# dominikbuenger/torch_nfft

Measured on AMD Instinct MI355X. Metric: Mpoints/s (adjoint+forward, 3-D N=256 m=4), higher is better.
Workload: dtype f32

## Files before the change

### torch_nfft_amd/csrc/colfft.hip

```cpp
#include <type_traits>

#include "common.h"
#include "kernels.h"

namespace nfft {

namespace {

constexpr int kFftThreads = 256;

struct ColGeom {
    int M, logM, N, H;
    int Mh;
    int SR;
    int KC;
    int KS;
    int NB;
    int NBm;
    int two_d;
    int NC, logNC;
    int TG;
    float param;
};

// ... 72 lines not shown
    static std::atomic<const float2 *> cache[kMaxDevices][7];
    const int dev = current_device();
    int slot = 0;
    while ((16 << slot) < M) ++slot;
    if (slot > 6 || (16 << slot) != M) return nullptr;
    if (dev < kMaxDevices) {
        const float2 *p = cache[dev][slot].load(std::memory_order_acquire);
        if (p) return p;
    }
    const float2 *p = nullptr;
    switch (M) {
    case 16: p = tw_symbol<16>(); break;
    case 32: p = tw_symbol<32>(); break;
    case 64: p = tw_symbol<64>(); break;
    case 128: p = tw_symbol<128>(); break;
    case 256: p = tw_symbol<256>(); break;
    case 512: p = tw_symbol<512>(); break;
    case 1024: p = tw_symbol<1024>(); break;
    }
    if (p && dev < kMaxDevices) cache[dev][slot].store(p, std::memory_order_release);
    return p;
}

__device__ __forceinline__ float2 cadd(float2 a, float2 b) { return make_float2(a.x + b.x, a.y + b.y); }
__device__ __forceinline__ float2 csub(float2 a, float2 b) { return make_float2(a.x - b.x, a.y - b.y); }
template <bool INV>
__device__ __forceinline__ float2 rot90(float2 a)
{
    return INV ? make_float2(-a.y, a.x) : make_float2(a.y, -a.x);
}

template <bool INV>
__device__ __forceinline__ void dft4(float2 &x0, float2 &x1, float2 &x2, float2 &x3)
{
    const float2 a0 = cadd(x0, x2), a1 = csub(x0, x2), a2 = cadd(x1, x3), a3 = rot90<INV>(csub(x1, x3));
    x0 = cadd(a0, a2);
    x1 = cadd(a1, a3);
    x2 = csub(a0, a2);
    x3 = csub(a1, a3);
}

template <bool INV>
__device__ __forceinline__ void dft8(float2 (&x)[8])
{
    dft4<INV>(x[0], x[2], x[4], x[6]);
    dft4<INV>(x[1], x[3], x[5], x[7]);
    constexpr float r = 0.70710678118654752440f;
    const float2 o0 = x[1];
    const float2 o1 = INV ? make_float2((x[3].x - x[3].y) * r, (x[3].x + x[3].y) * r)
                          : make_float2((x[3].x + x[3].y) * r, (x[3].y - x[3].x) * r);
    const float2 o2 = rot90<INV>(x[5]);
    const float2 o3 = INV ? make_float2((-x[7].x - x[7].y) * r, (x[7].x - x[7].y) * r)
                          : make_float2((x[7].y - x[7].x) * r, (-x[7].x - x[7].y) * r);
    const float2 e0 = x[0], e1 = x[2], e2 = x[4], e3 = x[6];
    x[0] = cadd(e0, o0); x[4] = csub(e0, o0);
    x[1] = cadd(e1, o1); x[5] = csub(e1, o1);
    x[2] = cadd(e2, o2); x[6] = csub(e2, o2);
    x[3] = cadd(e3, o3); x[7] = csub(e3, o3);
}

template <bool INV>
__device__ __forceinline__ float2 twiddle_at(const float2 *ltw, int e, int M)
{
    e &= M - 1;
    float2 w = ltw[e & (M / 2 - 1)];
    if (e >= M / 2) w = make_float2(-w.x, -w.y);
    if (INV) w.y = -w.y;
    return w;
}

template <bool INV, int R>
__device__ __forceinline__ void fft_stage(float2 *buf, const float2 *ltw, const ColGeom &cg, int tid, int logL)
{
    constexpr int logR = R == 8 ? 3 : 2;
    const int logLs = logL - logR, Ls = 1 << logLs;
    const int tstep = cg.M >> logL;
    const int total = (cg.M >> logR) << cg.logNC;
    __syncthreads();
    for (int idx = tid; idx < total; idx += kFftThreads) {
        const int col = idx & (cg.NC - 1);
        const int t = idx >> cg.logNC;
        const int j = t & (Ls - 1);
        const int row0 = ((t >> logLs) << logL) + j;
        float2 *p0 = buf + (row0 << cg.logNC) + col;
        const int stride = Ls << cg.logNC;
        float2 x[R];
#pragma unroll
        for (int q = 0; q < R; ++q) x[q] = p0[q * stride];
        if (R == 8) {
            dft8<INV>(reinterpret_cast<float2(&)[8]>(x));
        } else {
            dft4<INV>(x[0], x[1], x[2], x[3]);
        }
        p0[0] = x[0];
        if (logLs == 0) {
#pragma unroll
            for (int q = 1; q < R; ++q) p0[q * stride] = x[q];
        } else {
#pragma unroll
            for (int q = 1; q < R; ++q) p0[q * stride] = cmul(x[q], twiddle_at<INV>(ltw, j * q * tstep, cg.M));
        }
    }
}

template <bool INV>
__device__ __forceinline__ void lds_fft(float2 *buf, const float2 *ltw, const ColGeom &cg, int tid)
{
    switch (cg.logM) {
    case 4: fft_stage<INV, 4>(buf, ltw, cg, tid, 4); fft_stage<INV, 4>(buf, ltw, cg, tid, 2); break;
    case 5: fft_stage<INV, 8>(buf, ltw, cg, tid, 5); fft_stage<INV, 4>(buf, ltw, cg, tid, 2); break;
    case 6: fft_stage<INV, 8>(buf, ltw, cg, tid, 6); fft_stage<INV, 8>(buf, ltw, cg, tid, 3); break;
    case 7: fft_stage<INV, 8>(buf, ltw, cg, tid, 7); fft_stage<INV, 4>(buf, ltw, cg, tid, 4);
            fft_stage<INV, 4>(buf, ltw, cg, tid, 2); break;
    case 8: fft_stage<INV, 8>(buf, ltw, cg, tid, 8); fft_stage<INV, 8>(buf, ltw, cg, tid, 5);
            fft_stage<INV, 4>(buf, ltw, cg, tid, 2); break;
    case 9: fft_stage<INV, 8>(buf, ltw, cg, tid, 9); fft_stage<INV, 8>(buf, ltw, cg, tid, 6);
            fft_stage<INV, 8>(buf, ltw, cg, tid, 3); break;
    default: fft_stage<INV, 8>(buf, ltw, cg, tid, 10); fft_stage<INV, 8>(buf, ltw, cg, tid, 7);
             fft_stage<INV, 4>(buf, ltw, cg, tid, 4); fft_stage<INV, 4>(buf, ltw, cg, tid, 2); break;
    }
    __syncthreads();
}

__device__ __forceinline__ int brev_row(int k, int logM)
{
    int pos = 0, lg = logM;
    auto digit = [&](int lr) { lg -= lr; pos += (k & ((1 << lr) - 1)) << lg; k >>= lr; };
    switch (logM) {
    case 4: digit(2); digit(2); break;
    case 5: digit(3); digit(2); break;
    case 6: digit(3); digit(3); break;
    case 7: digit(3); digit(2); digit(2); break;
    case 8: digit(3); digit(3); digit(2); break;
    case 9: digit(3); digit(3); digit(3); break;
    default: digit(3); digit(3); digit(2); digit(2); break;
    }
    return pos;
}

template <int UN, typename LoadF, typename StoreF>
__device__ __forceinline__ void batched_fill(int total, int tid, LoadF load, StoreF store)
{
    for (int base = tid; base < total; base += kFftThreads * UN) {
        float2 v[UN];
#pragma unroll
        for (int r = 0; r < UN; ++r) {
            const int idx = base + r * kFftThreads;
            v[r] = idx < total ? load(idx) : make_float2(0.f, 0.f);
        }
#pragma unroll
        for (int r = 0; r < UN; ++r) {
            const int idx = base + r * kFftThreads;
            if (idx < total) store(idx, v[r]);
        }
    }
}

__device__ __forceinline__ void stage_twiddles(float2 *ltw, const float2 *__restrict__ tw, int M, int tid)
{
    for (int j = tid; j < M / 2; j += kFftThreads) ltw[j] = tw[j];
}

template <int LOGM, int LOGNC>
__global__ void __launch_bounds__(kFftThreads)
adj_axis1_kernel(ColGeom cg_in, const float2 *__restrict__ tw, const float2 *__restrict__ S, float2 *__restrict__ T)
{
    ColGeom cg = cg_in;
    if constexpr (LOGM > 0) {
        cg.M = 1 << LOGM;
        cg.logM = LOGM;
        cg.NC = 1 << LOGNC;
        cg.logNC = LOGNC;
    }
    extern __shared__ float2 smem[];
    float2 *ltw = smem;
    float2 *buf = smem + cg.M / 2;
    const int tid = threadIdx.x;
    int tile_x, u0;
    int64_t plane;
    column_tile_of_block(cg.TG, tile_x, u0, plane);
    const int c0 = tile_x << cg.logNC;
    if (c0 >= cg.KC) return;
    stage_twiddles(ltw, tw, cg.M, tid);
    const float2 *src = S + ((plane * cg.M + u0) * cg.M) * cg.SR;
    batched_fill<16>(cg.M << cg.logNC, tid,
                     [&](int idx) {
                         const int col = idx & (cg.NC - 1), u1 = idx >> cg.logNC;
                         const int k2 = c0 + col;
                         return k2 < cg.KC ? src[(int64_t)u1 * cg.SR + k2] : make_float2(0.f, 0.f);
                     },
                     [&](int idx, float2 v) { buf[idx] = v; });
    lds_fft<false>(buf, ltw, cg, tid);
    float2 *dst = T + ((plane * cg.M + u0) * cg.NB) * cg.KS;
    for (int idx = tid; idx < (cg.NB << cg.logNC); idx += kFftThreads) {
        const int col = idx & (cg.NC - 1), j1 = idx >> cg.logNC;
        const int k2 = c0 + col;
        if (k2 < cg.KC) {
            const int k1 = (j1 - cg.H) & (cg.M - 1);
            dst[(int64_t)j1 * cg.KS + k2] = buf[(brev_row(k1, cg.logM) << cg.logNC) + col];
        }
    }
}

__device__ __forceinline__ void apply_mult(const void *__restrict__ mult, int kind, int64_t f, float &re, float &im)
{
    if (kind == 1) {
        const float w = ((const float *)mult)[f];
        re *= w;
        im *= w;
    } else if (kind == 2) {
        const float2 w = ((const float2 *)mult)[f];
        const float r2 = re * w.x - im * w.y;
        im = re * w.y + im * w.x;
        re = r2;
    }
}

template <int LOGM, int LOGNC, bool XCOMPLEX, bool REAL_OUT>
__global__ void __launch_bounds__(kFftThreads)
adj_axis0_kernel(ColGeom cg_in, const float2 *__restrict__ tw, const float2 *__restrict__ T, int64_t C, int64_t col0,
                 void *__restrict__ yv, const void *__restrict__ mult, int mult_kind)
{
    ColGeom cg = cg_in;
    if constexpr (LOGM > 0) {
        cg.M = 1 << LOGM;
        cg.logM = LOGM;
        cg.NC = 1 << LOGNC;
        cg.logNC = LOGNC;
    }
    extern __shared__ float2 smem[];
    float2 *ltw = smem;
    float2 *buf = smem + cg.M / 2;
    float2 *buf2 = buf + (cg.M << cg.logNC);
    const int tid = threadIdx.x;
    int tile_x, j1;
    int64_t col_local;
    column_tile_of_block(cg.TG, tile_x, j1, col_local);
    const int c0 = tile_x << cg.logNC;
    if (c0 >= cg.KC) return;
    stage_twiddles(ltw, tw, cg.M, tid);
    const int64_t plane = XCOMPLEX ? col_local * 2 : col_local;
    const int64_t pstride = (int64_t)cg.M * cg.NBm * cg.KS;
    const float2 *src = T + plane * pstride + (int64_t)j1 * cg.KS;
    for (int part = 0; part < (XCOMPLEX ? 2 : 1); ++part) {
        float2 *const dstbuf = part ? buf2 : buf;
        const float2 *const srcp = src + part * pstride;
        batched_fill<16>(cg.M << cg.logNC, tid,
                         [&](int idx) {
                             const int col = idx & (cg.NC - 1), u0 = idx >> cg.logNC;
                             const int k2 = c0 + col;
                             return k2 < cg.KC ? srcp[(int64_t)u0 * cg.NBm * cg.KS + k2] : make_float2(0.f, 0.f);
                         },
                         [&](int idx, float2 v) { dstbuf[idx] = v; });
    }
    lds_fft<false>(buf, ltw, cg, tid);
    if (XCOMPLEX) lds_fft<false>(buf2, ltw, cg, tid);

    const int64_t colg = col0 + col_local;
    const int64_t b = colg / C, c = colg - b * C;
    const int H = cg.H, N = cg.N;
    const int k1 = cg.two_d ? 0 : j1 - H;
    const float f1 = cg.two_d ? 1.0f : phi_hat_inv_f(abs(k1), cg.param);
    const int64_t NN = cg.two_d ? (int64_t)N * N : (int64_t)N * N * N;
    for (int idx = tid; idx < (cg.NB << cg.logNC); idx += kFftThreads) {
        const int col = idx & (cg.NC - 1), j0 = idx >> cg.logNC;
        const int k2 = c0 + col;
        if (k2 >= cg.KC) continue;
        const int k0 = j0 - H;
        const int row = (brev_row(k0 & (cg.M - 1), cg.logM) << cg.logNC) + col;
        const float2 fr = buf[row];
        float2 fi = make_float2(0.f, 0.f);
        if (XCOMPLEX) fi = buf2[row];
        const float fac = phi_hat_inv_f(abs(k0), cg.param) * f1 * phi_hat_inv_f(k2, cg.param);
        if (k0 < H && k1 < H && k2 < H) {
            float re = (fr.x + fi.y) * fac, im = (-fr.y + fi.x) * fac;
            const int64_t f = cg.two_d ? (int64_t)(k0 + H) * N + (k2 + H) : ((int64_t)(k0 + H) * N + (k1 + H)) * N + (k2 + H);
            apply_mult(mult, mult_kind, f, re, im);
            const int64_t o = (b * NN + f) * C + c;
            if (REAL_OUT) ((float *)yv)[o] = re;
            else ((float2 *)yv)[o] = make_float2(re, im);
        }
        if (k2 >= 1 && k0 > -H && k1 > -H) {
            float re = (fr.x - fi.y) * fac, im = (fr.y + fi.x) * fac;
            const int64_t f = cg.two_d ? (int64_t)(H - k0) * N + (H - k2) : ((int64_t)(H - k0) * N + (H - k1)) * N + (H - k2);
            apply_mult(mult, mult_kind, f, re, im);
            const int64_t o = (b * NN + f) * C + c;
            if (REAL_OUT) ((float *)yv)[o] = re;
            else ((float2 *)yv)[o] = make_float2(re, im);
        }
    }
}

template <bool XCOMPLEX>
__device__ __forceinline__ float2 band_value(const void *__restrict__ xhat, int64_t b, int64_t c, int64_t C, int N,
                                             int H, int k0, int k1, int k2, const bool two_d = false)
{
    if (k0 < -H || k0 >= H || (!two_d && (k1 < -H || k1 >= H)) || k2 < -H || k2 >= H) return make_float2(0.f, 0.f);
    const int64_t idx = two_d ? ((b * N + (k0 + H)) * N + (k2 + H)) * C + c
                              : (((b * N + (k0 + H)) * N + (k1 + H)) * N + (k2 + H)) * C + c;
    if (XCOMPLEX) return ((const float2 *)xhat)[idx];
    return make_float2(((const float *)xhat)[idx], 0.f);
}

template <int LOGM, int LOGNC, bool XCOMPLEX>
__global__ void __launch_bounds__(kFftThreads)
fwd_axis0_kernel(ColGeom cg_in, const float2 *__restrict__ tw, const void *__restrict__ xhat, int64_t C, int ppc,
                 int64_t plane0, float2 *__restrict__ T)
{
    ColGeom cg = cg_in;
    if constexpr (LOGM > 0) {
        cg.M = 1 << LOGM;
        cg.logM = LOGM;
        cg.NC = 1 << LOGNC;
        cg.logNC = LOGNC;
    }
    extern __shared__ float2 smem[];
    float2 *ltw = smem;
    float2 *buf = smem + cg.M / 2;
    const int tid = threadIdx.x;
    int tile_x, j1;
    int64_t pl;
    column_tile_of_block(cg.TG, tile_x, j1, pl);
    const int c0 = tile_x << cg.logNC;
    if (c0 >= cg.KC) return;
    stage_twiddles(ltw, tw, cg.M, tid);
    for (int idx = tid; idx < (cg.M << cg.logNC); idx += kFftThreads) buf[idx] = make_float2(0.f, 0.f);
    __syncthreads();
    const int64_t plane = plane0 + pl;
    const int64_t colg = plane / ppc;
    const int part = (int)(plane - colg * ppc);
    const int64_t b = colg / C, c = colg - b * C;
    const int H = cg.H;
    const int k1 = cg.two_d ? 0 : j1 - H;
    const float f1 = cg.two_d ? 1.0f : phi_hat_inv_f(abs(k1), cg.param);
    batched_fill<8>(cg.NB << cg.logNC, tid,
                    [&](int idx) {
                        const int col = idx & (cg.NC - 1), j0 = idx >> cg.logNC;
                        const int k2 = c0 + col;
                        if (k2 >= cg.KC) return make_float2(0.f, 0.f);
                        const int k0 = j0 - H;
                        const float2 ap = band_value<XCOMPLEX>(xhat, b, c, C, cg.N, H, k0, k1, k2, cg.two_d != 0);
                        const float2 am = band_value<XCOMPLEX>(xhat, b, c, C, cg.N, H, -k0, -k1, -k2, cg.two_d != 0);
                        const float fac = 0.5f * phi_hat_inv_f(abs(k0), cg.param) * f1 * phi_hat_inv_f(k2, cg.param);
                        if (part == 0) return make_float2((am.x + ap.x) * fac, (am.y - ap.y) * fac);
                        return make_float2((am.y + ap.y) * fac, -(am.x - ap.x) * fac);
                    },
                    [&](int idx, float2 v) {
                        const int col = idx & (cg.NC - 1), j0 = idx >> cg.logNC;
                        if (c0 + col < cg.KC) buf[(((j0 - H) & (cg.M - 1)) << cg.logNC) + col] = v;
                    });
    lds_fft<true>(buf, ltw, cg, tid);
    float2 *dst = T + pl * ((int64_t)cg.M * cg.NBm * cg.KS) + (int64_t)j1 * cg.KS;
    for (int idx = tid; idx < (cg.M << cg.logNC); idx += kFftThreads) {
        const int col = idx & (cg.NC - 1), u0 = idx >> cg.logNC;
        const int k2 = c0 + col;
        if (k2 < cg.KC) dst[(int64_t)u0 * cg.NBm * cg.KS + k2] = buf[(brev_row(u0, cg.logM) << cg.logNC) + col];
    }
}

template <int LOGM, int LOGNC>
__global__ void __launch_bounds__(kFftThreads)
fwd_axis1_kernel(ColGeom cg_in, const float2 *__restrict__ tw, const float2 *__restrict__ T, float2 *__restrict__ S)
{
    ColGeom cg = cg_in;
    if constexpr (LOGM > 0) {
        cg.M = 1 << LOGM;
        cg.logM = LOGM;
        cg.NC = 1 << LOGNC;
        cg.logNC = LOGNC;
    }
    extern __shared__ float2 smem[];
    float2 *ltw = smem;
    float2 *buf = smem + cg.M / 2;
    const int tid = threadIdx.x;
    int tile_x, u0;
    int64_t plane;
    column_tile_of_block(cg.TG, tile_x, u0, plane);
    const int c0 = tile_x << cg.logNC;
    if (c0 >= (cg.SR == cg.KS ? cg.KC : cg.Mh)) return;
    float2 *dst = S + ((plane * cg.M + u0) * cg.M) * cg.SR;
    const int width = cg.SR == cg.KS ? cg.KC : cg.Mh;
    if (c0 >= cg.KC) {
        for (int idx = tid; idx < (cg.M << cg.logNC); idx += kFftThreads) {
            const int col = idx & (cg.NC - 1), u1 = idx >> cg.logNC;
            if (c0 + col < width) dst[(int64_t)u1 * cg.SR + c0 + col] = make_float2(0.f, 0.f);
        }
        return;
    }
    stage_twiddles(ltw, tw, cg.M, tid);
    for (int idx = tid; idx < (cg.M << cg.logNC); idx += kFftThreads) buf[idx] = make_float2(0.f, 0.f);
    __syncthreads();
    const float2 *src = T + ((plane * cg.M + u0) * cg.NB) * cg.KS;
    batched_fill<16>(cg.NB << cg.logNC, tid,
                     [&](int idx) {
                         const int col = idx & (cg.NC - 1), j1 = idx >> cg.logNC;
                         const int k2 = c0 + col;
                         return k2 < cg.KC ? src[(int64_t)j1 * cg.KS + k2] : make_float2(0.f, 0.f);
                     },
                     [&](int idx, float2 v) {
                         const int col = idx & (cg.NC - 1), j1 = idx >> cg.logNC;
                         if (c0 + col < cg.KC) buf[(((j1 - cg.H) & (cg.M - 1)) << cg.logNC) + col] = v;
                     });
    lds_fft<true>(buf, ltw, cg, tid);
    for (int idx = tid; idx < (cg.M << cg.logNC); idx += kFftThreads) {
        const int col = idx & (cg.NC - 1), u1 = idx >> cg.logNC;
        const int k2 = c0 + col;
        if (k2 < width) {
            dst[(int64_t)u1 * cg.SR + k2] =
                k2 < cg.KC ? buf[(brev_row(u1, cg.logM) << cg.logNC) + col] : make_float2(0.f, 0.f);
        }
    }
}

constexpr int kWaveCplx = 512;
constexpr int kRowWaves = 4;
constexpr int kR2cRounds = 1;
constexpr int kC2rRounds = 2;

__device__ __host__ constexpr int zsw(int i) { return i ^ ((i >> 3) & 0x1c) ^ ((i >> 2) & 3); }

template <bool INV, int R, int LOGLB, int LOGM>
__device__ __forceinline__ void wave_fft_stage(float2 *z, const float2 *ltw, int lane)
{
    constexpr int logR = R == 8 ? 3 : 2;
    constexpr int logLs = LOGLB - logR, Ls = 1 << logLs;
    constexpr int logT = LOGM - LOGLB;
    __builtin_amdgcn_wave_barrier();
#pragma unroll
    for (int t0 = 0; t0 < (kWaveCplx >> logR); t0 += 64) {
        const int t = t0 + lane;
        const int j = t & (Ls - 1);
        const int p0 = zsw(((t >> logLs) << LOGLB) + j);
        float2 x[R];
#pragma unroll
        for (int q = 0; q < R; ++q) x[q] = z[p0 ^ zsw(q * Ls)];
        if (R == 8) {
            dft8<INV>(reinterpret_cast<float2(&)[8]>(x));
        } else {
            dft4<INV>(x[0], x[1], x[2], x[3]);
        }
        z[p0] = x[0];
        if (logLs == 0) {
#pragma unroll
            for (int q = 1; q < R; ++q) z[p0 ^ zsw(q * Ls)] = x[q];
        } else {
            const int e1 = j << logT;
#pragma unroll
            for (int q = 1; q < R; ++q) {
                float2 w = ltw[(q * e1) & ((1 << LOGM) - 1)];
                if (INV) w.y = -w.y;
                z[p0 ^ zsw(q * Ls)] = cmul(x[q], w);
            }
        }
    }
    __builtin_amdgcn_wave_barrier();
}

template <bool INV, int LOGL>
__device__ __forceinline__ void wave_fft(float2 *z, const float2 *ltw, int lane)
{
    constexpr int LOGM = LOGL + 1;
    if constexpr (LOGL == 6) {
        wave_fft_stage<INV, 8, 6, LOGM>(z, ltw, lane); wave_fft_stage<INV, 8, 3, LOGM>(z, ltw, lane);
    } else if constexpr (LOGL == 7) {
        wave_fft_stage<INV, 8, 7, LOGM>(z, ltw, lane); wave_fft_stage<INV, 4, 4, LOGM>(z, ltw, lane);
        wave_fft_stage<INV, 4, 2, LOGM>(z, ltw, lane);
    } else if constexpr (LOGL == 8) {
        wave_fft_stage<INV, 8, 8, LOGM>(z, ltw, lane); wave_fft_stage<INV, 8, 5, LOGM>(z, ltw, lane);
        wave_fft_stage<INV, 4, 2, LOGM>(z, ltw, lane);
    } else {
        wave_fft_stage<INV, 8, 9, LOGM>(z, ltw, lane); wave_fft_stage<INV, 8, 6, LOGM>(z, ltw, lane);
        wave_fft_stage<INV, 8, 3, LOGM>(z, ltw, lane);
    }
}

template <int LOGL>
struct RowLds {
    float2 tw[2 << LOGL];
    float2 z[kRowWaves][kWaveCplx];
    unsigned short rev[1 << LOGL];
};

template <int LOGL>
__device__ __forceinline__ void row_tables(RowLds<LOGL> &S, const float2 *__restrict__ tw, int tid)
{
    constexpr int L = 1 << LOGL, M = 2 * L;
    for (int e = tid; e < M; e += kRowWaves * 64) {
        float2 w = tw[e & (L - 1)];
        if (e >= L) w = make_float2(-w.x, -w.y);
        S.tw[e] = w;
    }
    for (int k = tid; k < L; k += kRowWaves * 64) S.rev[k] = (unsigned short)brev_row(k, LOGL);
    __syncthreads();
}

template <int LOGL>
__global__ void __launch_bounds__(kRowWaves * 64)
row_r2c_kernel(int KC, int KS, int64_t nrows, const float2 *__restrict__ tw, const float *__restrict__ grid, float2 *__restrict__ out)
{
    constexpr int L = 1 << LOGL, M = 2 * L, RP = kWaveCplx / L;
    __shared__ RowLds<LOGL> S;
    const int tid = threadIdx.x, lane = tid & 63;
    const int wave = __builtin_amdgcn_readfirstlane(tid >> 6);
    float2 *z = S.z[wave];
    row_tables<LOGL>(S, tw, tid);
    const int64_t row0 = ((int64_t)blockIdx.x * kRowWaves + wave) * kR2cRounds * RP;
    float4 v4[kR2cRounds][kWaveCplx / 128];
#pragma unroll
    for (int r = 0; r < kR2cRounds; ++r) {
        const int64_t row = row0 + (int64_t)r * RP;
        const int nr = (int)max((int64_t)0, min((int64_t)RP, nrows - row));
        const float4 *src4 = (const float4 *)(grid + row * M);
#pragma unroll
        for (int q = 0; q < kWaveCplx / 128; ++q) {
            const int n2 = q * 64 + lane;
            v4[r][q] = 2 * n2 < nr * L ? src4[n2] : make_float4(0.f, 0.f, 0.f, 0.f);
        }
    }
#pragma unroll
    for (int r = 0; r < kR2cRounds; ++r) {
        const int64_t row = row0 + (int64_t)r * RP;
        if (row >= nrows) break;
        const int nr = (int)min((int64_t)RP, nrows - row);
#pragma unroll
        for (int q = 0; q < kWaveCplx / 128; ++q) {
            const int n2 = q * 64 + lane;
            z[zsw(2 * n2)] = make_float2(v4[r][q].x, v4[r][q].y);
            z[zsw(2 * n2 + 1)] = make_float2(v4[r][q].z, v4[r][q].w);
        }
        wave_fft<false, LOGL>(z, S.tw, lane);
        for (int rr = 0; rr < nr; ++rr) {
            float2 *dst = out + (row + rr) * KS;
            for (int k = lane; k < KC; k += 64) {
                const float2 a = z[zsw(rr * L + S.rev[k])];
                float2 b = z[zsw(rr * L + S.rev[(L - k) & (L - 1)])];
                b.y = -b.y;
                const float2 e = make_float2(0.5f * (a.x + b.x), 0.5f * (a.y + b.y));
                const float2 o = make_float2(0.5f * (a.x - b.x), 0.5f * (a.y - b.y));
                const float2 wo = cmul(S.tw[k], o);
                dst[k] = make_float2(e.x + wo.y, e.y - wo.x);
            }
        }
    }
}

template <int LOGL>
__global__ void __launch_bounds__(kRowWaves * 64)
row_c2r_kernel(int KC, int KS, int64_t nrows, const float2 *__restrict__ tw, const float2 *__restrict__ in, float *__restrict__ grid)
{
    constexpr int L = 1 << LOGL, M = 2 * L, RP = kWaveCplx / L;
    __shared__ RowLds<LOGL> S;
    const int tid = threadIdx.x, lane = tid & 63;
    const int wave = __builtin_amdgcn_readfirstlane(tid >> 6);
    float2 *z = S.z[wave];
    row_tables<LOGL>(S, tw, tid);
    const int64_t row0 = ((int64_t)blockIdx.x * kRowWaves + wave) * kC2rRounds * RP;
    constexpr int NIT = kWaveCplx / 64;
    float2 va[kC2rRounds][NIT];
#pragma unroll
    for (int r = 0; r < kC2rRounds; ++r) {
        const int64_t row = row0 + (int64_t)r * RP;
        const int nr = (int)max((int64_t)0, min((int64_t)RP, nrows - row));
        const float2 *src = in + row * KS;
#pragma unroll
        for (int it = 0; it < NIT; ++it) {
            const int n = it * 64 + lane;
            const int rr = n >> LOGL, k = n & (L - 1);
            const bool live = rr < nr;
            const int kk = k <= L / 2 ? k : L - k;
            va[r][it] = live ? src[rr * KS + kk] : make_float2(0.f, 0.f);
        }
    }
#pragma unroll
    for (int r = 0; r < kC2rRounds; ++r) {
        const int64_t row = row0 + (int64_t)r * RP;
        if (row >= nrows) break;
        const int nr = (int)min((int64_t)RP, nrows - row);
#pragma unroll
        for (int it = 0; it < NIT; ++it) {
            const int n = it * 64 + lane;
            const int k = n & (L - 1);
            const float2 v = va[r][it], zero = make_float2(0.f, 0.f);
            const float2 a = k <= L / 2 ? v : zero;
            float2 b = k >= L / 2 ? v : zero;
            b.y = -b.y;
            const float2 sum = make_float2(a.x + b.x, a.y + b.y), dif = make_float2(a.x - b.x, a.y - b.y);
            float2 w = S.tw[k];
            w.y = -w.y;
            const float2 wd = cmul(w, dif);
            z[zsw(n)] = make_float2(sum.x - wd.y, sum.y + wd.x);
        }
        wave_fft<true, LOGL>(z, S.tw, lane);
        float4 *dst4 = (float4 *)(grid + row * M);
#pragma unroll
        for (int q = 0; q < kWaveCplx / 128; ++q) {
            const int n2 = q * 64 + lane;
            const int na = 2 * n2, nb = 2 * n2 + 1;
            const int rr = na >> LOGL;
            if (rr < nr) {
                const float2 a = z[zsw(rr * L + S.rev[na & (L - 1)])], b = z[zsw(rr * L + S.rev[nb & (L - 1)])];
                dst4[n2] = make_float4(a.x, a.y, b.x, b.y);
            }
        }
    }
}

template <int LOGL>
__global__ void __launch_bounds__(kRowWaves * 64)
row_toeplitz_kernel(int KC, int KS, int64_t rows_per_plane, int64_t npairs, int64_t pair0, int64_t pairs_per_set,
                    const float2 *__restrict__ tw, const float *__restrict__ K, float2 *spec)
{
// ... 244 lines not shown
__global__ void __launch_bounds__(kFftThreads)
adj_axis0_ci_kernel(ColGeom cg, const float2 *__restrict__ tw, const float2 *__restrict__ T, int64_t C, int64_t plane0,
                    int64_t nplanes, void *__restrict__ yv, const void *__restrict__ mult, int mult_kind)
{
    extern __shared__ float2 smem[];
    float2 *ltw = smem;
    float2 *buf = smem + cg.M / 2;
    const int tid = threadIdx.x;
    const int k2 = blockIdx.x, j1 = blockIdx.y;
    const int64_t group = blockIdx.z;
    stage_twiddles(ltw, tw, cg.M, tid);
    const int64_t rs = (int64_t)cg.KC * kCiQ;
    const float2 *src = T + (group * cg.M * cg.NB + j1) * rs + (int64_t)k2 * kCiQ;
    batched_fill<16>(cg.M << kCiLogQ, tid,
                     [&](int idx) { return src[(int64_t)(idx >> kCiLogQ) * cg.NB * rs + (idx & (kCiQ - 1))]; },
                     [&](int idx, float2 v) { buf[idx] = v; });
    lds_fft<false>(buf, ltw, cg, tid);

    const int H = cg.H, N = cg.N;
    const int k1 = j1 - H;
    const float f12 = phi_hat_inv_f(abs(k1), cg.param) * phi_hat_inv_f(k2, cg.param);
    constexpr int PPC = XCOMPLEX ? 2 : 1;
    for (int idx = tid; idx < (cg.NB << kCiLogQ); idx += kFftThreads) {
        const int q = idx & (kCiQ - 1), j0 = idx >> kCiLogQ;
        if (XCOMPLEX && (q & 1)) continue;
        const int64_t pl = group * kCiQ + q;
        if (pl >= nplanes) continue;
        const int64_t colg = (plane0 + pl) / PPC;
        const int64_t b = colg / C, c = colg - b * C;
        const int k0 = j0 - H;
        const int row = (brev_row(k0 & (cg.M - 1), cg.logM) << kCiLogQ) + q;
        const float2 fr = buf[row];
        float2 fi = make_float2(0.f, 0.f);
        if (XCOMPLEX) fi = buf[row + 1];
        const float fac = phi_hat_inv_f(abs(k0), cg.param) * f12;
        if (k0 < H && k1 < H && k2 < H) {
            float re = (fr.x + fi.y) * fac, im = (-fr.y + fi.x) * fac;
            const int64_t f = ((int64_t)(k0 + H) * N + (k1 + H)) * N + (k2 + H);
            apply_mult(mult, mult_kind, f, re, im);
            const int64_t o = (b * N * N * N + f) * C + c;
            if (REAL_OUT) ((float *)yv)[o] = re;
            else ((float2 *)yv)[o] = make_float2(re, im);
        }
        if (k2 >= 1 && k0 > -H && k1 > -H) {
            float re = (fr.x - fi.y) * fac, im = (fr.y + fi.x) * fac;
            const int64_t f = ((int64_t)(H - k0) * N + (H - k1)) * N + (H - k2);
            apply_mult(mult, mult_kind, f, re, im);
            const int64_t o = (b * N * N * N + f) * C + c;
            if (REAL_OUT) ((float *)yv)[o] = re;
            else ((float2 *)yv)[o] = make_float2(re, im);
        }
    }
}

template <bool XCOMPLEX>
__global__ void __launch_bounds__(kFftThreads)
fwd_axis0_ci_kernel(ColGeom cg, const float2 *__restrict__ tw, const void *__restrict__ xhat, int64_t C, int ppc,
                    int64_t plane0, int64_t nplanes, float2 *__restrict__ T)
{
    extern __shared__ float2 smem[];
    float2 *ltw = smem;
    float2 *buf = smem + cg.M / 2;
    const int tid = threadIdx.x;
    const int k2 = blockIdx.x, j1 = blockIdx.y;
    const int64_t group = blockIdx.z;
    stage_twiddles(ltw, tw, cg.M, tid);
    for (int idx = tid; idx < (cg.M << kCiLogQ); idx += kFftThreads) buf[idx] = make_float2(0.f, 0.f);
    __syncthreads();
    const int H = cg.H;
    const int k1 = j1 - H;
    const float f12 = 0.5f * phi_hat_inv_f(abs(k1), cg.param) * phi_hat_inv_f(k2, cg.param);
    batched_fill<8>(cg.NB << kCiLogQ, tid,
                    [&](int idx) {
                        const int q = idx & (kCiQ - 1), j0 = idx >> kCiLogQ;
                        const int64_t pl = group * kCiQ + q;
                        if (pl >= nplanes) return make_float2(0.f, 0.f);
                        const int64_t plane = plane0 + pl;
                        const int64_t colg = plane / ppc;
                        const int part = (int)(plane - colg * ppc);
                        const int64_t b = colg / C, c = colg - b * C;
                        const int k0 = j0 - H;
                        const float2 ap = band_value<XCOMPLEX>(xhat, b, c, C, cg.N, H, k0, k1, k2);
                        const float2 am = band_value<XCOMPLEX>(xhat, b, c, C, cg.N, H, -k0, -k1, -k2);
                        const float fac = phi_hat_inv_f(abs(k0), cg.param) * f12;
                        if (part == 0) return make_float2((am.x + ap.x) * fac, (am.y - ap.y) * fac);
                        return make_float2((am.y + ap.y) * fac, -(am.x - ap.x) * fac);
                    },
                    [&](int idx, float2 v) {
                        const int q = idx & (kCiQ - 1), j0 = idx >> kCiLogQ;
                        buf[(((j0 - H) & (cg.M - 1)) << kCiLogQ) + q] = v;
                    });
    lds_fft<true>(buf, ltw, cg, tid);
    const int64_t rs = (int64_t)cg.KC * kCiQ;
    float2 *dst = T + (group * cg.M * cg.NB + j1) * rs + (int64_t)k2 * kCiQ;
    for (int idx = tid; idx < (cg.M << kCiLogQ); idx += kFftThreads) {
        const int q = idx & (kCiQ - 1), u0 = idx >> kCiLogQ;
        dst[(int64_t)u0 * cg.NB * rs + q] = buf[(brev_row(u0, cg.logM) << kCiLogQ) + q];
    }
}

__global__ void __launch_bounds__(kFftThreads)
fwd_axis1_ci_kernel(ColGeom cg, const float2 *__restrict__ tw, const float2 *__restrict__ T, float2 *__restrict__ S)
{
    extern __shared__ float2 smem[];
    float2 *ltw = smem;
    float2 *buf = smem + cg.M / 2;
    const int tid = threadIdx.x;
    const int k2 = blockIdx.x, u0 = blockIdx.y;
    const int64_t group = blockIdx.z;
    stage_twiddles(ltw, tw, cg.M, tid);
    for (int idx = tid; idx < (cg.M << kCiLogQ); idx += kFftThreads) buf[idx] = make_float2(0.f, 0.f);
    __syncthreads();
    const int64_t rs = (int64_t)cg.KC * kCiQ;
    const float2 *src = T + ((group * cg.M + u0) * cg.NB) * rs + (int64_t)k2 * kCiQ;
    batched_fill<16>(cg.NB << kCiLogQ, tid,
                     [&](int idx) { return src[(int64_t)(idx >> kCiLogQ) * rs + (idx & (kCiQ - 1))]; },
                     [&](int idx, float2 v) {
                         const int q = idx & (kCiQ - 1), j1 = idx >> kCiLogQ;
                         buf[(((j1 - cg.H) & (cg.M - 1)) << kCiLogQ) + q] = v;
                     });
    lds_fft<true>(buf, ltw, cg, tid);
    float2 *dst = S + ((group * cg.M + u0) * cg.M) * rs + (int64_t)k2 * kCiQ;
    for (int idx = tid; idx < (cg.M << kCiLogQ); idx += kFftThreads) {
        const int q = idx & (kCiQ - 1), u1 = idx >> kCiLogQ;
        dst[(int64_t)u1 * rs + q] = buf[(brev_row(u1, cg.logM) << kCiLogQ) + q];
    }
}

template <typename T, bool TO_INTERLEAVED>
__global__ void __launch_bounds__(256)
column_layout_kernel(const T *__restrict__ src, T *__restrict__ dst, int64_t K , int64_t C, int64_t col0,
                     int64_t ncols)
{
    __shared__ T tile[32][65];
    const int64_t k0 = (int64_t)blockIdx.x * 64;
    const int64_t cl0 = (int64_t)blockIdx.y * 32;
    const int tid = threadIdx.x;
    if (TO_INTERLEAVED) {
        for (int e = tid; e < 32 * 64; e += 256) {
            const int cl = e >> 6, k = e & 63;
            if (cl0 + cl < ncols && k0 + k < K) tile[cl][k] = src[(cl0 + cl) * K + k0 + k];
        }
        __syncthreads();
        for (int e = tid; e < 32 * 64; e += 256) {
            const int k = e >> 5, cl = e & 31;
            if (cl0 + cl < ncols && k0 + k < K) {
                const int64_t colg = col0 + cl0 + cl, b = colg / C, c = colg - b * C;
                dst[(b * K + k0 + k) * C + c] = tile[cl][k];
            }
        }
    } else {
        for (int e = tid; e < 32 * 64; e += 256) {
            const int k = e >> 5, cl = e & 31;
            if (cl0 + cl < ncols && k0 + k < K) {
                const int64_t colg = col0 + cl0 + cl, b = colg / C, c = colg - b * C;
                tile[cl][k] = src[(b * K + k0 + k) * C + c];
            }
        }
        __syncthreads();
        for (int e = tid; e < 32 * 64; e += 256) {
            const int cl = e >> 6, k = e & 63;
            if (cl0 + cl < ncols && k0 + k < K) dst[(cl0 + cl) * K + k0 + k] = tile[cl][k];
        }
    }
}

int compact_stride(const Geom &g)
{
    const int a = g.M >= 512 ? 8 : 4;
    return (g.N / 2 + 1 + a - 1) / a * a;
}

ColGeom make_col_geom(const Geom &g, bool two_buffers, bool compact, int64_t planes = 0)
{
    ColGeom cg;
    cg.M = g.M;
    cg.logM = 0;
    while ((1 << cg.logM) < g.M) ++cg.logM;
    cg.N = g.N;
    cg.H = g.N / 2;
    cg.Mh = g.M / 2 + 1;
    cg.KC = cg.H + 1;
    cg.KS = compact_stride(g);
    cg.SR = compact ? cg.KS : cg.Mh;
    cg.NB = g.N + 1;
    cg.two_d = g.dim == 2;
    cg.NBm = cg.two_d ? 1 : cg.NB;
    int nc = 16;
    const int64_t cap = g.M >= 1024 ? 65536 : 32768;
    while (nc > 1 && (int64_t)g.M * nc * 8 * (two_buffers ? 2 : 1) > cap) nc >>= 1;
    if (g.dim == 2 && planes > 0)
        while (nc > 4 && ((g.N / 2 + 1 + nc - 1) / nc) * planes < 64) nc >>= 1;
    cg.NC = nc;
    cg.logNC = 0;
    while ((1 << cg.logNC) < nc) ++cg.logNC;
    cg.param = g.rolloff ? 1.047197551196597746f * (float)g.m / ((float)g.N * (float)g.N) : 0.0f;
    cg.TG = nc >= 16 ? 1 : 16 / nc;
    return cg;
}

static inline unsigned col_tiles(const ColGeom &cg, int columns = 0)
{
    const int t = ((columns > 0 ? columns : cg.KC) + cg.NC - 1) / cg.NC;
    return (unsigned)((t + cg.TG - 1) / cg.TG * cg.TG);
}

size_t col_lds_bytes(const ColGeom &cg, bool two_buffers)
{
    return (size_t)(cg.M / 2 + (int64_t)cg.M * cg.NC * (two_buffers ? 2 : 1)) * sizeof(float2);
}

template <typename K>
void allow_lds(K kernel, size_t bytes)
{
    if (bytes > 48 * 1024) (void)hipFuncSetAttribute((const void *)kernel, hipFuncAttributeMaxDynamicSharedMemorySize, (int)bytes);
}

}

bool colfft_supported(const Geom &g)
{
    if (g.dim == 2) return g.M >= 128 && g.M <= 1024 && (g.M & (g.M - 1)) == 0;
    return g.dim == 3 && g.M >= 16 && g.M <= 1024 && (g.M & (g.M - 1)) == 0;
}

int64_t colfft_scratch_bytes(const Geom &g, int64_t nplanes)
{
    return align_up(nplanes * (int64_t)g.M * (g.dim == 2 ? 1 : g.N + 1) * compact_stride(g) * 8, 256) + align_up((int64_t)g.M * 4, 256);
}

template <typename F>
static void col_dispatch(const ColGeom &cg, F &&f)
{
    using std::integral_constant;
    if (cg.logM == 9 && cg.logNC == 3) return f(integral_constant<int, 9>{}, integral_constant<int, 3>{});
    if (cg.logM == 9 && cg.logNC == 2) return f(integral_constant<int, 9>{}, integral_constant<int, 2>{});
    return f(integral_constant<int, 0>{}, integral_constant<int, 0>{});
}

int launch_colfft_adjoint(const Geom &g, const float2 *spec, bool compact, void *scratch, int64_t scratch_planes,
                          int64_t C, int x_is_complex, int real_output, int64_t plane0, int64_t nplanes, void *y,
                          const void *mult, int mult_kind, hipStream_t stream)
{
    if (nplanes <= 0) return 0;
    const float2 *T = (const float2 *)scratch;
    const float2 *tw = twiddle_table(g.M);
    if (!tw) { set_error("no twiddle table for this grid size"); return 4; }
    if (g.dim == 2) {
        if (!compact) { set_error("2-D column passes need the compact half spectrum of the own row passes"); return 4; }
        T = spec;
    } else {
        const ColGeom cg = make_col_geom(g, false, compact);
        const dim3 grid(col_tiles(cg), g.M, (unsigned)nplanes);
        const size_t lds = col_lds_bytes(cg, false);
        col_dispatch(cg, [&](auto lm, auto ln) {
            constexpr int LM = decltype(lm)::value, LN = decltype(ln)::value;
            allow_lds(adj_axis1_kernel<LM, LN>, lds);
            hipLaunchKernelGGL((adj_axis1_kernel<LM, LN>), grid, dim3(kFftThreads), lds, stream, cg, tw, spec, (float2 *)scratch);
        });
    }
    {
        const bool two = x_is_complex != 0;
        const int ppc = two ? 2 : 1;
        const int64_t col0 = plane0 / ppc, ncols = nplanes / ppc;
        const ColGeom cg = make_col_geom(g, two, compact, ncols);
        const dim3 grid(col_tiles(cg), cg.NBm, (unsigned)ncols);
        const size_t lds = col_lds_bytes(cg, two);
        col_dispatch(cg, [&](auto lm, auto ln) {
            constexpr int LM = decltype(lm)::value, LN = decltype(ln)::value;
            auto go = [&](auto kernel) {
                allow_lds(kernel, lds);
                hipLaunchKernelGGL(kernel, grid, dim3(kFftThreads), lds, stream, cg, tw, T, C, col0, y, mult, mult_kind);
            };
            if (two) {
                if (real_output) go(adj_axis0_kernel<LM, LN, true, true>);
                else go(adj_axis0_kernel<LM, LN, true, false>);
            } else {
                if (real_output) go(adj_axis0_kernel<LM, LN, false, true>);
                else go(adj_axis0_kernel<LM, LN, false, false>);
            }
        });
    }
    NFFT_HIP_CHECK(hipGetLastError());
    return 0;
}

int launch_colfft_forward(const Geom &g, const void *xhat, void *scratch, int64_t scratch_planes, int64_t C,
                          int x_is_complex, int real_output, int64_t plane0, int64_t nplanes, float2 *spec, bool compact,
                          hipStream_t stream)
{
    if (nplanes <= 0) return 0;
    float2 *T = (float2 *)scratch;
    const float2 *tw = twiddle_table(g.M);
    if (!tw) { set_error("no twiddle table for this grid size"); return 4; }
    if (g.dim == 2) {
        if (!compact) { set_error("2-D column passes need the compact half spectrum of the own row passes"); return 4; }
        T = spec;
    }
    const ColGeom cg = make_col_geom(g, false, compact, nplanes);
    const size_t lds = col_lds_bytes(cg, false);
    const int ppc = real_output ? 1 : 2;
    col_dispatch(cg, [&](auto lm, auto ln) {
        constexpr int LM = decltype(lm)::value, LN = decltype(ln)::value;
        {
            const dim3 grid(col_tiles(cg), cg.NBm, (unsigned)nplanes);
            if (x_is_complex) {
                allow_lds(fwd_axis0_kernel<LM, LN, true>, lds);
                hipLaunchKernelGGL((fwd_axis0_kernel<LM, LN, true>), grid, dim3(kFftThreads), lds, stream, cg, tw, xhat, C, ppc, plane0, T);
            } else {
                allow_lds(fwd_axis0_kernel<LM, LN, false>, lds);
                hipLaunchKernelGGL((fwd_axis0_kernel<LM, LN, false>), grid, dim3(kFftThreads), lds, stream, cg, tw, xhat, C, ppc, plane0, T);
            }
        }
        if (g.dim != 2) {
            const dim3 grid(col_tiles(cg, compact ? cg.KC : cg.Mh), g.M, (unsigned)nplanes);
            allow_lds(fwd_axis1_kernel<LM, LN>, lds);
            hipLaunchKernelGGL((fwd_axis1_kernel<LM, LN>), grid, dim3(kFftThreads), lds, stream, cg, tw, T, spec);
        }
    });
    NFFT_HIP_CHECK(hipGetLastError());
    return 0;
}

bool colfft_ci_supported(const Geom &g) { return g.dim == 3 && colfft_supported(g) && g.M >= 128 && g.M <= 1024; }

int64_t colfft_ci_planes(int64_t nplanes) { return (nplanes + kCiQ - 1) / kCiQ * kCiQ; }

static ColGeom make_ci_geom(const Geom &g)
{
    ColGeom cg = make_col_geom(g, false, true);
    cg.NC = kCiQ;
    cg.logNC = kCiLogQ;
    return cg;
}

template <int LOGL>
static int launch_rows_ci_t(bool c2r, const Geom &g, int64_t nplanes, const float2 *tw, const void *in, void *out,
                            hipStream_t stream)
{
    constexpr int RP = kWaveCplx >> LOGL;
    const int64_t rows = (int64_t)g.M * g.M;
    const dim3 blocks((unsigned)(rows / RP), (unsigned)((nplanes + kCiQ - 1) / kCiQ));
    const size_t lds = sizeof(RowCiLds<LOGL>);
    static DeviceOnce attr_done;
    if (attr_done.first_use()) {
        NFFT_HIP_CHECK(hipFuncSetAttribute((const void *)row_r2c_ci_kernel<LOGL>, hipFuncAttributeMaxDynamicSharedMemorySize, (int)lds));
        NFFT_HIP_CHECK(hipFuncSetAttribute((const void *)row_c2r_ci_kernel<LOGL>, hipFuncAttributeMaxDynamicSharedMemorySize, (int)lds));
        attr_done.mark();
    }
    if (c2r)
        hipLaunchKernelGGL((row_c2r_ci_kernel<LOGL>), blocks, dim3(kCiQ * 64), lds, stream, rows, nplanes, tw, (const float2 *)in,
                           (float *)out);
    else
        hipLaunchKernelGGL((row_r2c_ci_kernel<LOGL>), blocks, dim3(kCiQ * 64), lds, stream, rows, nplanes, tw, (const float *)in,
                           (float2 *)out);
    NFFT_HIP_CHECK(hipGetLastError());
    return 0;
}

static int launch_rows_ci(bool c2r, const Geom &g, int64_t nplanes, const void *in, void *out, hipStream_t stream)
{
    if (nplanes <= 0) return 0;
    const float2 *tw = twiddle_table(g.M);
    if (!tw) { set_error("no twiddle table for this grid size"); return 4; }
    switch (g.M) {
    case 128: return launch_rows_ci_t<6>(c2r, g, nplanes, tw, in, out, stream);
    case 256: return launch_rows_ci_t<7>(c2r, g, nplanes, tw, in, out, stream);
    case 512: return launch_rows_ci_t<8>(c2r, g, nplanes, tw, in, out, stream);
    case 1024: return launch_rows_ci_t<9>(c2r, g, nplanes, tw, in, out, stream);
    }
    set_error("row passes support M = 128 .. 1024");
    return 1;
}

int launch_row_r2c_ci(const Geom &g, const float *grid, int64_t nplanes, float2 *spec, hipStream_t stream)
{
    return launch_rows_ci(false, g, nplanes, grid, spec, stream);
}
int launch_row_c2r_ci(const Geom &g, const float2 *spec, int64_t nplanes, float *grid, hipStream_t stream)
{
    return launch_rows_ci(true, g, nplanes, spec, grid, stream);
}

int launch_colfft_adjoint_ci(const Geom &g, const float2 *spec, void *scratch, int64_t C, int x_is_complex,
                             int real_output, int64_t plane0, int64_t nplanes, void *y, const void *mult, int mult_kind,
                             hipStream_t stream)
{
    if (nplanes <= 0) return 0;
    float2 *T = (float2 *)scratch;
    const float2 *tw = twiddle_table(g.M);
    if (!tw) { set_error("no twiddle table for this grid size"); return 4; }
    const ColGeom cg = make_ci_geom(g);
    const size_t lds = col_lds_bytes(cg, false);
    const unsigned groups = (unsigned)((nplanes + kCiQ - 1) / kCiQ);
    allow_lds(adj_axis1_ci_kernel, lds);
    hipLaunchKernelGGL(adj_axis1_ci_kernel, dim3(cg.KC, g.M, groups), dim3(kFftThreads), lds, stream, cg, tw, spec, T);
    auto go = [&](auto kernel) {
        allow_lds(kernel, lds);
        hipLaunchKernelGGL(kernel, dim3(cg.KC, cg.NB, groups), dim3(kFftThreads), lds, stream, cg, tw, T, C, plane0, nplanes, y,
                           mult, mult_kind);
    };
    if (x_is_complex) {
        if (real_output) go(adj_axis0_ci_kernel<true, true>);
        else go(adj_axis0_ci_kernel<true, false>);
    } else {
        if (real_output) go(adj_axis0_ci_kernel<false, true>);
        else go(adj_axis0_ci_kernel<false, false>);
    }
    NFFT_HIP_CHECK(hipGetLastError());
    return 0;
}

void colfft_tile_widths(const Geom &g, bool compact, bool ci, int x_is_complex, int64_t nplanes, int32_t *out)
{
    const bool two = x_is_complex != 0;
    const ColGeom geoms[3] = {ci ? make_ci_geom(g) : make_col_geom(g, false, compact),
                              ci ? make_ci_geom(g) : make_col_geom(g, two, compact, nplanes / (two ? 2 : 1)),
                              ci ? make_ci_geom(g) : make_col_geom(g, false, compact, nplanes)};
    for (int i = 0; i < 3; ++i) {
        int specialised = 0;
        if (!ci) col_dispatch(geoms[i], [&](auto lm, auto) { specialised = decltype(lm)::value != 0; });
        out[2 * i] = geoms[i].NC;
        out[2 * i + 1] = specialised;
    }
    if (g.dim == 2) out[0] = out[1] = 0;
}

int launch_colfft_forward_ci(const Geom &g, const void *xhat, float2 *spec, void *scratch, int64_t C, int x_is_complex,
                             int real_output, int64_t plane0, int64_t nplanes, hipStream_t stream)
{
    if (nplanes <= 0) return 0;
    float2 *T = (float2 *)scratch;
    const float2 *tw = twiddle_table(g.M);
    if (!tw) { set_error("no twiddle table for this grid size"); return 4; }
    const ColGeom cg = make_ci_geom(g);
    const size_t lds = col_lds_bytes(cg, false);
    const unsigned groups = (unsigned)((nplanes + kCiQ - 1) / kCiQ);
    const int ppc = real_output ? 1 : 2;
    if (x_is_complex) {
        allow_lds(fwd_axis0_ci_kernel<true>, lds);
        hipLaunchKernelGGL((fwd_axis0_ci_kernel<true>), dim3(cg.KC, cg.NB, groups), dim3(kFftThreads), lds, stream, cg, tw, xhat, C,
                           ppc, plane0, nplanes, T);
    } else {
        allow_lds(fwd_axis0_ci_kernel<false>, lds);
        hipLaunchKernelGGL((fwd_axis0_ci_kernel<false>), dim3(cg.KC, cg.NB, groups), dim3(kFftThreads), lds, stream, cg, tw, xhat, C,
                           ppc, plane0, nplanes, T);
    }
    allow_lds(fwd_axis1_ci_kernel, lds);
    hipLaunchKernelGGL(fwd_axis1_ci_kernel, dim3(cg.KC, g.M, groups), dim3(kFftThreads), lds, stream, cg, tw, T, spec);
    NFFT_HIP_CHECK(hipGetLastError());
    return 0;
}

bool rowfft_supported(const Geom &g)
{
    return colfft_supported(g) && g.M >= 128 && g.M <= 1024;
}

template <int LOGL>
static void launch_rows_t(bool c2r, const Geom &g, int64_t nrows, const float2 *tw, const void *in, void *out,
                          hipStream_t stream)
{
    const int64_t per_wg = (int64_t)kRowWaves * (c2r ? kC2rRounds : kR2cRounds) * (kWaveCplx >> LOGL);
    const dim3 blocks((unsigned)((nrows + per_wg - 1) / per_wg));
    if (c2r)
        hipLaunchKernelGGL((row_c2r_kernel<LOGL>), blocks, dim3(kRowWaves * 64), 0, stream, g.N / 2 + 1, compact_stride(g), nrows, tw,
                           (const float2 *)in, (float *)out);
    else
        hipLaunchKernelGGL((row_r2c_kernel<LOGL>), blocks, dim3(kRowWaves * 64), 0, stream, g.N / 2 + 1, compact_stride(g), nrows, tw,
                           (const float *)in, (float2 *)out);
}

static int launch_rows(bool c2r, const Geom &g, int64_t nplanes, const float2 *tw, const void *in, void *out,
                       hipStream_t stream)
{
    const int64_t nrows = nplanes * g.Ma[0] * g.Ma[1];
    switch (g.M) {
    case 128: launch_rows_t<6>(c2r, g, nrows, tw, in, out, stream); break;
    case 256: launch_rows_t<7>(c2r, g, nrows, tw, in, out, stream); break;
    case 512: launch_rows_t<8>(c2r, g, nrows, tw, in, out, stream); break;
    case 1024: launch_rows_t<9>(c2r, g, nrows, tw, in, out, stream); break;
    default: set_error("row passes support M = 128 .. 1024"); return 1;
    }
    NFFT_HIP_CHECK(hipGetLastError());
    return 0;
}

int launch_row_r2c(const Geom &g, const float *grid, void *scratch, int64_t scratch_planes, int64_t nplanes,
                   float2 *spec, hipStream_t stream)
{
    if (nplanes <= 0) return 0;
    const float2 *tw = twiddle_table(g.M);
    if (!tw) { set_error("no twiddle table for this grid size"); return 4; }
    return launch_rows(false, g, nplanes, tw, grid, spec, stream);
}

int launch_row_c2r(const Geom &g, const float2 *spec, void *scratch, int64_t scratch_planes, int64_t nplanes,
                   float *grid, hipStream_t stream)
{
    if (nplanes <= 0) return 0;
    const float2 *tw = twiddle_table(g.M);
    if (!tw) { set_error("no twiddle table for this grid size"); return 4; }
    return launch_rows(true, g, nplanes, tw, spec, grid, stream);
}

template <int LOGL>
static void launch_row_toeplitz_t(const Geom &g, const float2 *tw, float2 *spec, const float *K, int64_t pairs_per_set,
                                  int64_t pair0, int64_t npairs, hipStream_t stream)
{
    const int64_t rows_per_plane = (int64_t)g.Ma[0] * g.Ma[1];
    const int64_t units = npairs * (rows_per_plane / (kWaveCplx >> LOGL));
    const dim3 blocks((unsigned)((units + kRowWaves - 1) / kRowWaves));
    hipLaunchKernelGGL((row_toeplitz_kernel<LOGL>), blocks, dim3(kRowWaves * 64), 0, stream, g.N / 2 + 1, compact_stride(g),
                       rows_per_plane, npairs, pair0, pairs_per_set, tw, K, spec);
}

int launch_row_toeplitz(const Geom &g, float2 *spec, const float *K, int64_t pairs_per_set, int64_t pair0, int64_t npairs,
                        hipStream_t stream)
{
    if (npairs <= 0) return 0;
    const float2 *tw = twiddle_table(g.M);
    if (!tw) { set_error("no twiddle table for this grid size"); return 4; }
    switch (g.M) {
    case 128: launch_row_toeplitz_t<6>(g, tw, spec, K, pairs_per_set, pair0, npairs, stream); break;
    case 256: launch_row_toeplitz_t<7>(g, tw, spec, K, pairs_per_set, pair0, npairs, stream); break;
    case 512: launch_row_toeplitz_t<8>(g, tw, spec, K, pairs_per_set, pair0, npairs, stream); break;
    case 1024: launch_row_toeplitz_t<9>(g, tw, spec, K, pairs_per_set, pair0, npairs, stream); break;
    default: set_error("row passes support M = 128 .. 1024"); return 1;
    }
    NFFT_HIP_CHECK(hipGetLastError());
    return 0;
}

int launch_column_layout(bool to_interleaved, const void *src, void *dst, int64_t K, int64_t C, int64_t col0,
                         int64_t ncols, int elem_bytes, hipStream_t stream)
{
    if (ncols <= 0 || K <= 0) return 0;
    const dim3 blocks((unsigned)((K + 63) / 64), (unsigned)((ncols + 31) / 32));
    if (elem_bytes == 8) {
        if (to_interleaved)
            hipLaunchKernelGGL((column_layout_kernel<float2, true>), blocks, dim3(256), 0, stream, (const float2 *)src,
                               (float2 *)dst, K, C, col0, ncols);
        else
            hipLaunchKernelGGL((column_layout_kernel<float2, false>), blocks, dim3(256), 0, stream, (const float2 *)src,
                               (float2 *)dst, K, C, col0, ncols);
    } else {
        if (to_interleaved)
            hipLaunchKernelGGL((column_layout_kernel<float, true>), blocks, dim3(256), 0, stream, (const float *)src,
                               (float *)dst, K, C, col0, ncols);
        else
            hipLaunchKernelGGL((column_layout_kernel<float, false>), blocks, dim3(256), 0, stream, (const float *)src,
                               (float *)dst, K, C, col0, ncols);
    }
    NFFT_HIP_CHECK(hipGetLastError());
    return 0;
}

}
```

Before: 2899.

## Specialize forward axis-0 column FFT for M=512 with prefetched register loads

Adds a fixed-size path of the forward axis-0 column kernel for the case where half the grid size equals the thread count. It issues all band loads into registers up front, before staging twiddles and zeroing LDS, so global latency overlaps that setup. It also uses a 1-D grid with 32-bit offsets and specialized fill logic in place of the generic per-element bounds checks. A size guard falls back to the generic kernel when offsets could overflow 32 bits; the cost is more register use and code duplication.

```diff
diff --git a/torch_nfft_amd/csrc/colfft.hip b/torch_nfft_amd/csrc/colfft.hip
--- a/torch_nfft_amd/csrc/colfft.hip
+++ b/torch_nfft_amd/csrc/colfft.hip
@@ -398,11 +398,110 @@
     return make_float2(((const float *)xhat)[idx], 0.f);
 }
 
+__device__ __forceinline__ float2 hermitian_part(float2 ap, float2 am, float fac, int part)
+{
+    if (part == 0) return make_float2((am.x + ap.x) * fac, (am.y - ap.y) * fac);
+    return make_float2((am.y + ap.y) * fac, -(am.x - ap.x) * fac);
+}
+
+__device__ __forceinline__ bool in_band(int H, int k0, int k1, int k2, const bool two_d)
+{
+    return !(k0 < -H || k0 >= H || (!two_d && (k1 < -H || k1 >= H)) || k2 < -H || k2 >= H);
+}
+
+template <int LOGM, int LOGNC, bool XCOMPLEX>
+__device__ __forceinline__ void fwd_axis0_fixed(ColGeom cg, const float2 *__restrict__ tw, const void *__restrict__ xhat, int64_t C,
+                                                int ppc, int64_t plane0, float2 *__restrict__ T)
+{
+    using E = std::conditional_t<XCOMPLEX, float2, float>;
+    constexpr int M = 1 << LOGM, NC = 1 << LOGNC, N = M / 2, NB = N + 1;
+    constexpr int FILL = NB * NC, UE = (FILL + kFftThreads - 1) / kFftThreads;
+    constexpr int RS = kFftThreads >> LOGNC;
+    static_assert(RS * (UE - 1) == N, "the last round of the fill is row j0 = N alone");
+    cg.M = M;
+    cg.logM = LOGM;
+    cg.NC = NC;
+    cg.logNC = LOGNC;
+    extern __shared__ float2 smem[];
+    float2 *ltw = smem;
+    float2 *buf = smem + M / 2;
+    const int tid = threadIdx.x;
+    const unsigned tiles = (unsigned)((cg.KC + NC - 1) >> LOGNC), q = blockIdx.x / tiles;
+    const int c0 = (int)(blockIdx.x - q * tiles) << LOGNC, j1 = (int)(q % (unsigned)cg.NBm);
+    const int64_t pl = (int64_t)(q / (unsigned)cg.NBm);
+    const int64_t plane = plane0 + pl;
+    const int64_t colg = plane / ppc;
+    const int part = (int)(plane - colg * ppc);
+    const int64_t b = colg / C, c = colg - b * C;
+    const int H = cg.H;
+    const bool two_d = cg.two_d != 0;
+    const E *const X = (const E *)xhat + b * (two_d ? (int64_t)N * N : (int64_t)N * N * N) * C + c;
+    const float2 twv = tw[tid];
+    E vp[UE], vm[UE];
+    {
+        const int Ci = (int)C, rowC = (two_d ? N : N * N) * Ci;
+        const int r0 = tid >> LOGNC, k2 = c0 + (tid & (NC - 1));
+        const bool up = two_d || j1 < N, um = two_d || j1 > 0;
+        const int inner_p = two_d ? (k2 + H) * Ci : (j1 * N + k2 + H) * Ci;
+        const int inner_m = two_d ? (H - k2) * Ci : ((N - j1) * N + H - k2) * Ci;
+        const bool lane_m = um && k2 < cg.KC;
+        const unsigned offp = up && k2 < H ? (unsigned)(r0 * rowC + inner_p) : 0u;
+        const unsigned offm = lane_m ? (unsigned)((RS - r0) * rowC + inner_m) : 0u;
+#pragma unroll
+        for (int e = 0; e < UE - 1; ++e) {
+            vp[e] = (X + (up ? e * RS * rowC : 0))[offp];
+            vm[e] = (X + (um ? (N - (e + 1) * RS) * rowC : 0))[e == 0 && r0 == 0 ? 0u : offm];
+        }
+        vp[UE - 1] = E{};
+        vm[UE - 1] = X[lane_m && r0 == 0 ? (unsigned)inner_m : 0u];
+    }
+    asm volatile("" ::: "memory");
+    ltw[tid] = twv;
+    for (int i = tid; i < (M - NB) * NC; i += kFftThreads) buf[((H + 1) << LOGNC) + i] = make_float2(0.f, 0.f);
+    const int k1 = two_d ? 0 : j1 - H;
+    const float f1 = two_d ? 1.0f : phi_hat_inv_f(abs(k1), cg.param);
+#pragma unroll
+    for (int e = 0; e < UE; ++e) {
+        const int idx = tid + e * kFftThreads;
+        if (idx >= FILL) continue;
+        const int col = idx & (NC - 1), j0 = idx >> LOGNC;
+        const int k2 = c0 + col, k0 = j0 - H;
+        float2 ap = make_float2(0.f, 0.f), am = make_float2(0.f, 0.f);
+        if constexpr (XCOMPLEX) {
+            if (in_band(H, k0, k1, k2, two_d)) ap = vp[e];
+            if (in_band(H, -k0, -k1, -k2, two_d)) am = vm[e];
+        } else {
+            if (in_band(H, k0, k1, k2, two_d)) ap.x = vp[e];
+            if (in_band(H, -k0, -k1, -k2, two_d)) am.x = vm[e];
+        }
+        const float fac = 0.5f * phi_hat_inv_f(abs(k0), cg.param) * f1 * phi_hat_inv_f(k2, cg.param);
+        const float2 val = hermitian_part(ap, am, fac, part);
+        buf[(((j0 - H) & (M - 1)) << LOGNC) + col] = k2 < cg.KC ? val : make_float2(0.f, 0.f);
+    }
+    lds_fft<true>(buf, ltw, cg, tid);
+    float2 *dst = T + pl * ((int64_t)M * cg.NBm * cg.KS) + (int64_t)j1 * cg.KS;
+    for (int idx = tid; idx < M * NC; idx += kFftThreads) {
+        const int col = idx & (NC - 1), u0 = idx >> LOGNC;
+        const int k2 = c0 + col;
+        if (k2 < cg.KC) dst[(int64_t)u0 * cg.NBm * cg.KS + k2] = buf[(brev_row(u0, LOGM) << LOGNC) + col];
+    }
+}
+
+template <int LOGM>
+constexpr bool fwd_axis0_is_fixed()
+{
+    return LOGM > 0 && (1 << LOGM) / 2 == kFftThreads;
+}
+
 template <int LOGM, int LOGNC, bool XCOMPLEX>
 __global__ void __launch_bounds__(kFftThreads)
 fwd_axis0_kernel(ColGeom cg_in, const float2 *__restrict__ tw, const void *__restrict__ xhat, int64_t C, int ppc,
                  int64_t plane0, float2 *__restrict__ T)
 {
+    if constexpr (fwd_axis0_is_fixed<LOGM>()) {
+        fwd_axis0_fixed<LOGM, LOGNC, XCOMPLEX>(cg_in, tw, xhat, C, ppc, plane0, T);
+        return;
+    }
     ColGeom cg = cg_in;
     if constexpr (LOGM > 0) {
         cg.M = 1 << LOGM;
@@ -1253,16 +1352,23 @@
     const int ppc = real_output ? 1 : 2;
     col_dispatch(cg, [&](auto lm, auto ln) {
         constexpr int LM = decltype(lm)::value, LN = decltype(ln)::value;
-        {
+        auto axis0 = [&](auto xc) {
+            constexpr bool XC = decltype(xc)::value;
+            if constexpr (fwd_axis0_is_fixed<LM>()) {
+                if ((g.dim == 2 ? (int64_t)g.N * g.N : (int64_t)g.N * g.N * g.N) * C < (1ll << 30)) {
+                    const dim3 grid((unsigned)((int64_t)((cg.KC + cg.NC - 1) / cg.NC) * cg.NBm * nplanes));
+                    allow_lds(fwd_axis0_kernel<LM, LN, XC>, lds);
+                    hipLaunchKernelGGL((fwd_axis0_kernel<LM, LN, XC>), grid, dim3(kFftThreads), lds, stream, cg, tw, xhat, C, ppc, plane0, T);
+                    return;
+                }
+            }
+            constexpr int RM = fwd_axis0_is_fixed<LM>() ? 0 : LM, RN = fwd_axis0_is_fixed<LM>() ? 0 : LN;
             const dim3 grid(col_tiles(cg), cg.NBm, (unsigned)nplanes);
-            if (x_is_complex) {
-                allow_lds(fwd_axis0_kernel<LM, LN, true>, lds);
-                hipLaunchKernelGGL((fwd_axis0_kernel<LM, LN, true>), grid, dim3(kFftThreads), lds, stream, cg, tw, xhat, C, ppc, plane0, T);
-            } else {
-                allow_lds(fwd_axis0_kernel<LM, LN, false>, lds);
-                hipLaunchKernelGGL((fwd_axis0_kernel<LM, LN, false>), grid, dim3(kFftThreads), lds, stream, cg, tw, xhat, C, ppc, plane0, T);
-            }
-        }
+            allow_lds(fwd_axis0_kernel<RM, RN, XC>, lds);
+            hipLaunchKernelGGL((fwd_axis0_kernel<RM, RN, XC>), grid, dim3(kFftThreads), lds, stream, cg, tw, xhat, C, ppc, plane0, T);
+        };
+        if (x_is_complex) axis0(std::true_type{});
+        else axis0(std::false_type{});
         if (g.dim != 2) {
             const dim3 grid(col_tiles(cg, compact ? cg.KC : cg.Mh), g.M, (unsigned)nplanes);
             allow_lds(fwd_axis1_kernel<LM, LN>, lds);
```

New measurement: 2907 (median of 4 runs). No clear change (+0.3%).
